# yuriyvnv/speech_transcript_embeddings

Measured on AMD Instinct MI355X. Metric: audio–text pairs/sec (whole node), 10s@16kHz + 64-tok, 1/2/4/8 MI355X, higher is better.
Workload: dtype bf16; 1 GPU; c2: global batch 64 = 1 GPU x 1 micro-batch(es) of 64 pairs, each pair 10s@16kHz audio + 64-tok clean + 64-tok corrupt; w2v-bert-2.0 Conformer 24L + XLM-R-base 12L, 3+3 unfrozen; GPU fbank -> fwd -> InfoNCE -> bwd -> allreduce -> clip+AdamW; global_batch=64, local_batch=64, micro_batch=64, accumulation_steps=1, seq_len_audio_frames=499, seq_len_text=64, parallelism=dp1

## Files before the change

include/ste.h:

```cpp
#ifndef STE_H_
#define STE_H_
#include <stdint.h>

#ifdef __cplusplus
extern "C" {
#endif

#define STE_OK 0
#define STE_ERR_ARG 1001
#define STE_ERR_SHAPE 1002

enum {
  STE_ACT_NONE = 0,
  STE_ACT_SWISH = 1,
  STE_ACT_GELU = 2,
  STE_ACT_TANH = 3,
  STE_ACT_RELU = 4,
  STE_ACT_SWISH_BWD = 11,
  STE_ACT_GELU_BWD = 12,
  STE_ACT_TANH_BWD_OUT = 13,
  STE_ACT_RELU_BWD = 14
};

typedef struct {
// ... 61 lines not shown
  const void* dy; int64_t lddy; int dy_bf16;
  const void* x; int64_t ldx; int x_bf16;
  const float* mean; const float* rstd;
  const float* gamma; const float* beta;
  const float* row_scale;
  int act;
  const float* dres; int64_t lddres;
  float* dx; int64_t lddx;
  void* dxb; int64_t lddxb;
  float* dgamma; float* dbeta;
  float drop_p; uint64_t seed; float out_scale;
  float in_drop_p; uint64_t in_seed;
  const float* out_row_scale;
  float* dsum;
  float* ws; int64_t ws_floats;
} ste_ln_bwd_args;
int ste_layernorm_bwd(const ste_ln_bwd_args* a, void* stream);
int64_t ste_layernorm_bwd_ws_floats(int rows, int cols);

int ste_layernorm_fwd_pair(const ste_ln_fwd_args* a, const ste_ln_fwd_args* b, void* stream);
int ste_layernorm_bwd_pair(const ste_ln_bwd_args* a, const ste_ln_bwd_args* b, void* stream);

typedef struct {
  int B, T, H;
  const void* q; int64_t ldq;
  const void* k; int64_t ldk;
  const void* v; int64_t ldv;
  void* o; int64_t ldo;
  float* lse;
  const int32_t* key_mask;
  const void* rel_E; int rel_left, rel_right;
  float scale;
  float drop_p; uint64_t seed;
  const void* dout; int64_t lddo;
  void* dq; int64_t lddq;
  void* dk; int64_t lddk;
  void* dv; int64_t lddv;
  float* delta;
  float* dE;
  float* gwork;
  void* o_lo; int64_t ldolo;
  int zero_masked_rows;
} ste_attn_args;
int ste_attention_fwd(const ste_attn_args* a, void* stream);
int ste_attention_fwd_f32(const ste_attn_args* a, float* o32, int64_t ldo32, void* stream);
int ste_attention_bwd(const ste_attn_args* a, void* stream);
int ste_attention_bwd_f32(const ste_attn_args* a, void* stream);

int ste_glu_dwconv_fwd(const void* pre, const float* w, void* out, int B, int T, int C, int K, void* stream);
int ste_glu_dwconv_bwd(const void* pre, const float* w, const void* dout, void* dpre, float* dw,
                       int B, int T, int C, int K, float* ws, int64_t ws_floats, void* stream);
int64_t ste_glu_dwconv_bwd_ws_floats(int B, int T, int C, int K);

int ste_fbank(const float* wav, int64_t ld_wav, const int32_t* lengths, int B, int Tmax, float pad_value,
              float* feats, int64_t* mask, int mask_mode, float* work, void* stream);

int ste_resample_plan(int sr_in, int sr_out, int* M, int* L, int* K);
int ste_resample_table(int sr_in, int sr_out, float* table, int64_t table_floats);
int ste_resample_tile(int M, int L, int K);
int ste_resample(const float* wav, int64_t ld_wav, const int32_t* lengths, int B, int M, int L, int K,
                 const float* table, float* out, int64_t ld_out, int n_out_max, int32_t* out_lengths, void* stream);

int ste_attn_pool_fwd(const void* t, const float* w2, const float* b2, const void* h, const int32_t* mask,
                      int B, int L, int Hh, int H, float* weights, float* pooled, void* pooled_bf16,
                      void* stream);
int ste_attn_pool_bwd_work_floats(int B, int L, int Hh);
int ste_attn_pool_bwd(const void* t, const float* w2, const void* h, const float* weights, const float* dpooled,
                      const int32_t* mask, int B, int L, int Hh, int H, float* dh, void* dt, void* dt_lo, float* dw2,
                      float* db2,
                      float* db1, float* work, void* stream);
int ste_attn_pool_fwd_f32(const float* t, const float* w2, const float* b2, const float* h, const int32_t* mask,
                          int B, int L, int Hh, int H, float* weights, float* pooled, void* pooled_bf16, void* stream);
int ste_attn_pool_bwd_f32(const float* t, const float* w2, const float* h, const float* weights, const float* dpooled,
                          const int32_t* mask, int B, int L, int Hh, int H, float* dh, float* dt, float* dw2,
                          float* db2, float* db1, float* work, void* stream);

int ste_mean_pool_fwd(const void* h, const int32_t* mask, int B, int L, int H, int cls, float* weights, float* pooled,
                      void* pooled_bf16, void* stream);
int ste_mean_pool_fwd_f32(const float* h, const int32_t* mask, int B, int L, int H, int cls, float* weights,
                          float* pooled, void* pooled_bf16, void* stream);
int ste_weighted_pool_bwd(const float* weights, const float* dpooled, int B, int L, int H, float* dh, void* stream);

int ste_xattn1_fwd(const float* q, const void* k, const void* v, int64_t ldkv, const int32_t* mask, int B, int S,
                   int P, int nh, float scale, float drop_p, uint64_t seed, float* probs, float* out, void* stream);
int ste_xattn1_bwd(const float* q, const void* k, const void* v, int64_t ldkv, const float* probs, const float* dout,
                   const int32_t* mask, int B, int S, int P, int nh, float scale, float drop_p, uint64_t seed,
                   float* dq, float* dk, float* dv, int64_t lddkv, void* stream);
int ste_xattn_fwd(const float* q, const void* k, const void* v, int64_t ldkv, const int32_t* mask, int B, int S, int P,
                  int nh, int nq, float scale, float drop_p, uint64_t seed0, uint64_t seed1, float* probs, float* out,
                  void* stream);
int ste_xattn_bwd(const float* q, const void* k, const void* v, int64_t ldkv, const float* probs, const float* dout,
                  const int32_t* mask, int B, int S, int P, int nh, int nq, float scale, float drop_p,
                  uint64_t seed0, uint64_t seed1, float* dq, float* dk, float* dv, int64_t lddkv, void* stream);
int ste_xattn_mq_fwd(const float* q, const int32_t* qrow, const void* k, const void* v, int64_t ldkv,
                     const int32_t* mask, int B, int C, int S, int P, int nh, float scale, float* out, void* stream);
int ste_xattn_gather_fwd(const float* q, const int32_t* qrow, const void* k, const void* v, int64_t ldkv,
                         const int32_t* kvblk, const int32_t* mask, int R, int S, int P, int nh, float scale,
                         float* out, void* stream);
int ste_xattn_seg_fwd(const float* q, const int32_t* qrow, const int32_t* pseg, const void* k, const void* v,
                      int64_t ldkv, const int64_t* seg_row, const int32_t* seg_len, const int32_t* tile_first,
                      const int32_t* tile_cnt, int ntile, int R, int G, int P, int nh, float scale, float* out,
                      void* stream);
int ste_xattn_seg_mx8_fwd(const float* q, const int32_t* qrow, const int32_t* pseg, const void* k, const void* v,
                          int64_t ldkv, const void* ks, const void* vs, int64_t lds, const int64_t* seg_row,
                          const int32_t* seg_len, const int32_t* tile_first, const int32_t* tile_cnt, int ntile,
                          int R, int G, int P, int nh, float scale, float* out, void* stream);
// ... 140 lines not shown
```

speech_transcript_embeddings_amd/_lib.py:

```python
from __future__ import annotations

import ctypes as C
import os
from pathlib import Path

import torch

_PKG = Path(__file__).resolve().parent
LIB_PATH = Path(os.environ.get("STE_LIB", _PKG / "libste.so"))
AB_BUILD = LIB_PATH.name == "libste_ab.so"


def ab_env(name: str, default: str) -> str:
    return os.environ.get(name, default) if AB_BUILD else default

c_void_p, c_int, c_int64, c_float, c_uint64, c_char_p = C.c_void_p, C.c_int, C.c_int64, C.c_float, C.c_uint64, C.c_char_p
c_i32p = C.POINTER(C.c_int32)

ACT_NONE, ACT_SWISH, ACT_GELU, ACT_TANH, ACT_RELU = 0, 1, 2, 3, 4
ACT_SWISH_BWD, ACT_GELU_BWD, ACT_TANH_BWD_OUT, ACT_RELU_BWD = 11, 12, 13, 14


class GemmArgs(C.Structure):
    _fields_ = [
# ... 58 lines not shown
    _fields_ = [
        ("B", c_int), ("T", c_int), ("H", c_int),
        ("q", c_void_p), ("ldq", c_int64),
        ("k", c_void_p), ("ldk", c_int64),
        ("v", c_void_p), ("ldv", c_int64),
        ("o", c_void_p), ("ldo", c_int64),
        ("lse", c_void_p),
        ("key_mask", c_void_p),
        ("rel_E", c_void_p), ("rel_left", c_int), ("rel_right", c_int),
        ("scale", c_float),
        ("drop_p", c_float), ("seed", c_uint64),
        ("dout", c_void_p), ("lddo", c_int64),
        ("dq", c_void_p), ("lddq", c_int64),
        ("dk", c_void_p), ("lddk", c_int64),
        ("dv", c_void_p), ("lddv", c_int64),
        ("delta", c_void_p),
        ("dE", c_void_p),
        ("gwork", c_void_p),
        ("o_lo", c_void_p), ("ldolo", c_int64),
        ("zero_masked_rows", c_int),
    ]


_SIGS = {
    "ste_gemm": (c_int, [C.POINTER(GemmArgs), c_void_p]),
    "ste_gemm_f32": (c_int, [C.POINTER(GemmArgs), c_void_p]),
    "ste_gemm_f32_plan": (c_int, [C.POINTER(GemmArgs)]),
    "ste_gemm_f32_plan_slab": (c_int, [C.POINTER(GemmArgs)]),
    "ste_gemm_f32_ws_floats": (c_int64, [C.POINTER(GemmArgs)]),
    "ste_gemm_f32_plan_max_tiles": (c_int, [c_int]),
    "ste_gemm_f32_plan_small_tiles": (c_int, [c_int]),
    "ste_gemm_f32_plan_tile": (c_int, [C.POINTER(GemmArgs)]),
    "ste_gemm_kernel": (c_int, [C.POINTER(GemmArgs)]),
    "ste_gemm_colsum_ws_floats": (c_int64, [C.POINTER(GemmArgs)]),
    "ste_gemm_tile_map": (c_int, [c_int, c_int, c_int, C.POINTER(c_int), C.POINTER(c_int)]),
    "ste_gemm_kernel_name": (c_int, [C.POINTER(GemmArgs), c_char_p, c_int]),
    "ste_rows_extract": (c_int, [c_void_p, c_int, c_int, c_void_p, c_int, c_void_p, c_void_p, c_void_p, c_int,
                                 c_void_p, c_void_p]),
    "ste_rows_accumulate": (c_int, [c_void_p, c_int, c_void_p, c_void_p, c_int, c_float, c_void_p]),
    "ste_layernorm_fwd": (c_int, [C.POINTER(LnFwdArgs), c_void_p]),
    "ste_layernorm_bwd": (c_int, [C.POINTER(LnBwdArgs), c_void_p]),
    "ste_layernorm_fwd_pair": (c_int, [C.POINTER(LnFwdArgs), C.POINTER(LnFwdArgs), c_void_p]),
    "ste_layernorm_bwd_pair": (c_int, [C.POINTER(LnBwdArgs), C.POINTER(LnBwdArgs), c_void_p]),
    "ste_layernorm_bwd_ws_floats": (c_int64, [c_int, c_int]),
    "ste_attention_fwd": (c_int, [C.POINTER(AttnArgs), c_void_p]),
    "ste_attention_bwd": (c_int, [C.POINTER(AttnArgs), c_void_p]),
    "ste_attention_fwd_f32": (c_int, [C.POINTER(AttnArgs), c_void_p, c_int64, c_void_p]),
    "ste_attention_bwd_f32": (c_int, [C.POINTER(AttnArgs), c_void_p]),
    "ste_split_bf16": (c_int, [c_void_p, c_int64, c_int64, c_int, c_void_p, c_int, c_int, c_void_p]),
    "ste_glu_dwconv_fwd": (c_int, [c_void_p, c_void_p, c_void_p, c_int, c_int, c_int, c_int, c_void_p]),
    "ste_glu_dwconv_bwd": (c_int, [c_void_p, c_void_p, c_void_p, c_void_p, c_void_p, c_int, c_int, c_int, c_int,
                                   c_void_p, c_int64, c_void_p]),
    "ste_glu_dwconv_bwd_ws_floats": (c_int64, [c_int, c_int, c_int, c_int]),
    "ste_fbank": (c_int, [c_void_p, c_int64, c_void_p, c_int, c_int, c_float, c_void_p, c_void_p, c_int, c_void_p,
                          c_void_p]),
    "ste_resample_plan": (c_int, [c_int, c_int, C.POINTER(c_int), C.POINTER(c_int), C.POINTER(c_int)]),
    "ste_resample_table": (c_int, [c_int, c_int, c_void_p, c_int64]),
    "ste_resample_tile": (c_int, [c_int, c_int, c_int]),
    "ste_resample": (c_int, [c_void_p, c_int64, c_void_p, c_int, c_int, c_int, c_int, c_void_p, c_void_p, c_int64,
                             c_int, c_void_p, c_void_p]),
    "ste_gemm_mx8": (c_int, [c_void_p, c_void_p, c_void_p, c_void_p, c_void_p, c_void_p]),
    "ste_gemm_mx8_kernel": (c_int, [C.POINTER(GemmArgs), c_int]),
    "ste_gemm_plan_min_tiles": (c_int, [c_int, c_int, C.POINTER(c_int), C.POINTER(c_int)]),
    "ste_mx8_quant": (c_int, [c_void_p, c_int64, c_int, c_int, c_void_p, c_void_p, c_void_p]),
    "ste_mx8_dequant": (c_int, [c_void_p, c_int64, c_int, c_int, c_void_p, c_void_p, c_void_p]),
    "ste_attn_pool_fwd": (c_int, [c_void_p, c_void_p, c_void_p, c_void_p, c_void_p, c_int, c_int, c_int, c_int,
                                  c_void_p, c_void_p, c_void_p, c_void_p]),
    "ste_attn_pool_bwd": (c_int, [c_void_p, c_void_p, c_void_p, c_void_p, c_void_p, c_void_p, c_int, c_int, c_int,
                                  c_int, c_void_p, c_void_p, c_void_p, c_void_p, c_void_p, c_void_p, c_void_p,
                                  c_void_p]),
    "ste_attn_pool_bwd_work_floats": (c_int, [c_int, c_int, c_int]),
    "ste_attn_pool_fwd_f32": (c_int, [c_void_p, c_void_p, c_void_p, c_void_p, c_void_p, c_int, c_int, c_int, c_int,
                                      c_void_p, c_void_p, c_void_p, c_void_p]),
    "ste_attn_pool_bwd_f32": (c_int, [c_void_p, c_void_p, c_void_p, c_void_p, c_void_p, c_void_p, c_int, c_int,
                                      c_int, c_int, c_void_p, c_void_p, c_void_p, c_void_p, c_void_p, c_void_p,
                                      c_void_p]),
    "ste_mean_pool_fwd": (c_int, [c_void_p, c_void_p, c_int, c_int, c_int, c_int, c_void_p, c_void_p, c_void_p,
                                  c_void_p]),
    "ste_mean_pool_fwd_f32": (c_int, [c_void_p, c_void_p, c_int, c_int, c_int, c_int, c_void_p, c_void_p, c_void_p,
                                      c_void_p]),
    "ste_weighted_pool_bwd": (c_int, [c_void_p, c_void_p, c_int, c_int, c_int, c_void_p, c_void_p]),
    "ste_xattn1_fwd": (c_int, [c_void_p, c_void_p, c_void_p, c_int64, c_void_p, c_int, c_int, c_int, c_int, c_float,
                               c_float, c_uint64, c_void_p, c_void_p, c_void_p]),
    "ste_xattn1_bwd": (c_int, [c_void_p, c_void_p, c_void_p, c_int64, c_void_p, c_void_p, c_void_p, c_int, c_int,
                               c_int, c_int, c_float, c_float, c_uint64, c_void_p, c_void_p, c_void_p, c_int64,
                               c_void_p]),
    "ste_xattn_fwd": (c_int, [c_void_p, c_void_p, c_void_p, c_int64, c_void_p, c_int, c_int, c_int, c_int, c_int,
                              c_float, c_float, c_uint64, c_uint64, c_void_p, c_void_p, c_void_p]),
    "ste_xattn_bwd": (c_int, [c_void_p, c_void_p, c_void_p, c_int64, c_void_p, c_void_p, c_void_p, c_int, c_int,
                              c_int, c_int, c_int, c_float, c_float, c_uint64, c_uint64, c_void_p, c_void_p,
                              c_void_p, c_int64, c_void_p]),
    "ste_xattn_bwd_bf16": (c_int, [c_void_p, c_void_p, c_void_p, c_int64, c_void_p, c_void_p, c_void_p, c_int,
                                   c_int, c_int, c_int, c_int, c_float, c_float, c_uint64, c_uint64, c_void_p,
                                   c_void_p, c_void_p, c_int64, c_void_p, c_void_p]),
    "ste_xattn_mq_fwd": (c_int, [c_void_p, c_void_p, c_void_p, c_void_p, c_int64, c_void_p, c_int, c_int, c_int,
                                 c_int, c_int, c_float, c_void_p, c_void_p]),
    "ste_xattn_gather_fwd": (c_int, [c_void_p, c_void_p, c_void_p, c_void_p, c_int64, c_void_p, c_void_p, c_int,
                                     c_int, c_int, c_int, c_float, c_void_p, c_void_p]),
    "ste_xattn_seg_fwd": (c_int, [c_void_p, c_void_p, c_void_p, c_void_p, c_void_p, c_int64, c_void_p, c_void_p,
                                  c_void_p, c_void_p, c_int, c_int, c_int, c_int, c_int, c_float, c_void_p,
                                  c_void_p]),
    "ste_xattn_seg_mx8_fwd": (c_int, [c_void_p, c_void_p, c_void_p, c_void_p, c_void_p, c_int64, c_void_p, c_void_p,
                                      c_int64, c_void_p, c_void_p, c_void_p, c_void_p, c_int, c_int, c_int, c_int,
                                      c_int, c_float, c_void_p, c_void_p]),
    "ste_align_attn_fwd": (c_int, [c_void_p, c_int64, c_void_p, c_int64, c_void_p, c_int, c_int, c_int, c_int, c_int,
                                   c_float, c_uint64, c_void_p, c_void_p, c_int64, c_void_p]),
# ... 138 lines not shown
```

speech_transcript_embeddings_amd/csrc/layernorm.hip:

```cpp
#include "common.h"
#include "../../include/ste.h"

namespace {

constexpr int NT = 256;

template <int MAXC>
STE_DEV void load_row(const void* base, bool is_bf16, int64_t ld, int row, int cols, int lane, float (&v)[MAXC * 4]) {
#pragma unroll
  for (int c = 0; c < MAXC; ++c) {
    int col = (lane + c * 64) * 4;
    f32x4 x = {0.f, 0.f, 0.f, 0.f};
    if (col < cols) {
      if (is_bf16) x = load_bf16x4((const bf16*)base + (int64_t)row * ld + col);
      else x = *reinterpret_cast<const f32x4*>((const float*)base + (int64_t)row * ld + col);
    }
#pragma unroll
    for (int e = 0; e < 4; ++e) v[c * 4 + e] = x[e];
  }
}

template <int MAXC>
struct LnParams {
  f32x4 g[MAXC], b[MAXC];
  STE_DEV void load(const float* gamma, const float* beta, int cols, int lane) {
#pragma unroll
    for (int c = 0; c < MAXC; ++c) {
      const int col = (lane + c * 64) * 4;
      g[c] = col < cols ? *reinterpret_cast<const f32x4*>(gamma + col) : f32x4{0.f, 0.f, 0.f, 0.f};
      b[c] = (beta && col < cols) ? *reinterpret_cast<const f32x4*>(beta + col) : f32x4{0.f, 0.f, 0.f, 0.f};
    }
  }
};

template <int MAXC>
STE_DEV void ln_fwd_row(const ste_ln_fwd_args& a, const LnParams<MAXC>& pr, int row, int lane, float (&v)[MAXC * 4]) {
  const float inv_n = 1.0f / (float)a.cols;
  const uint32_t thresh = (uint32_t)(a.drop_p * 4294967296.0);
  const float inv_keep = a.drop_p > 0.f ? 1.0f / (1.0f - a.drop_p) : 1.0f;
  float s = 0.f;
#pragma unroll
  for (int i = 0; i < MAXC * 4; ++i) s += v[i];
  const float mean = wave_sum(s) * inv_n;
  float q = 0.f;
#pragma unroll
  for (int c = 0; c < MAXC; ++c) {
    int col = (lane + c * 64) * 4;
    if (col < a.cols) {
#pragma unroll
      for (int e = 0; e < 4; ++e) { float d = v[c * 4 + e] - mean; q += d * d; }
    }
  }
  const float rstd = rsqrtf(wave_sum(q) * inv_n + a.eps);
  if (lane == 0) { a.mean[row] = mean; a.rstd[row] = rstd; }
  const float rs = a.row_scale ? a.row_scale[row] : 1.0f;
#pragma unroll
  for (int c = 0; c < MAXC; ++c) {
    int col = (lane + c * 64) * 4;
    if (col >= a.cols) continue;
    const f32x4 g = pr.g[c], b = pr.b[c];
    f32x4 y;
#pragma unroll
    for (int e = 0; e < 4; ++e) {
      float t = ((v[c * 4 + e] - mean) * rstd * g[e] + b[e]) * rs;
      if (a.act == STE_ACT_SWISH) t = swish_f(t);
      if (a.drop_p > 0.f) t *= drop_scale(a.seed, (uint64_t)row * a.cols + col + e, thresh, inv_keep);
      y[e] = t;
      v[c * 4 + e] = t;
    }
    if (a.y) *reinterpret_cast<f32x4*>(a.y + (int64_t)row * a.ldy + col) = y;
    if (a.ylo) store_bf16x4_split((bf16*)a.yb + (int64_t)row * a.ldyb + col, (bf16*)a.ylo + (int64_t)row * a.ldylo + col, y);
    else if (a.yb) store_bf16x4((bf16*)a.yb + (int64_t)row * a.ldyb + col, y);
    if (a.q8) {
      float am = fmaxf(fmaxf(fabsf(y[0]), fabsf(y[1])), fmaxf(fabsf(y[2]), fabsf(y[3])));
      am = fmaxf(am, dpp_f<0xB1>(am));
      am = fmaxf(am, dpp_f<0x4E>(am));
      am = fmaxf(am, dpp_f<0x141>(am));
      const int ex = mx8_exp(am);
      const float inv = ldexpf(1.0f, -ex);
      uint32_t w = 0;
      w = __builtin_amdgcn_cvt_pk_fp8_f32(fminf(fmaxf(y[0] * inv, -448.f), 448.f),
                                          fminf(fmaxf(y[1] * inv, -448.f), 448.f), w, false);
      w = __builtin_amdgcn_cvt_pk_fp8_f32(fminf(fmaxf(y[2] * inv, -448.f), 448.f),
                                          fminf(fmaxf(y[3] * inv, -448.f), 448.f), w, true);
      *reinterpret_cast<uint32_t*>((uint8_t*)a.q8 + (int64_t)row * a.ldq8 + col) = w;
      if ((lane & 7) == 0) ((uint8_t*)a.q8s)[(int64_t)row * (a.cols >> 5) + (col >> 5)] = (uint8_t)(ex + 127);
    }
  }
}

template <int MAXC>
__global__ __launch_bounds__(NT) void ln_fwd_kernel(ste_ln_fwd_args a) {
  const int lane = threadIdx.x & 63;
  const int wave = blockIdx.x * (NT / 64) + (threadIdx.x >> 6);
  const int nwaves = gridDim.x * (NT / 64);
  LnParams<MAXC> pa;
  pa.load(a.gamma, a.beta, a.cols, lane);
  for (int row = wave; row < a.rows; row += nwaves) {
    float v[MAXC * 4];
    load_row<MAXC>(a.x, a.x_bf16, a.ldx, row, a.cols, lane, v);
    ln_fwd_row<MAXC>(a, pa, row, lane, v);
  }
}

template <int MAXC, bool LEAN = false>
__global__ __launch_bounds__(NT) void ln_fwd_pair_kernel(ste_ln_fwd_args a, ste_ln_fwd_args b) {
  const int lane = threadIdx.x & 63;
  const int wave = blockIdx.x * (NT / 64) + (threadIdx.x >> 6);
  const int nwaves = gridDim.x * (NT / 64);
  if constexpr (LEAN) {
    for (int row = wave; row < a.rows; row += nwaves) {
      float v[MAXC * 4];
      load_row<MAXC>(a.x, a.x_bf16, a.ldx, row, a.cols, lane, v);
      const float *ga = a.gamma, *ba = a.beta, *gb = b.gamma, *bb = b.beta;
      asm volatile("" : "+s"(ga), "+s"(ba), "+s"(gb), "+s"(bb));
      {
        LnParams<MAXC> pa;
        pa.load(ga, ba, a.cols, lane);
        ln_fwd_row<MAXC>(a, pa, row, lane, v);
      }
      LnParams<MAXC> pb;
      pb.load(gb, bb, b.cols, lane);
      ln_fwd_row<MAXC>(b, pb, row, lane, v);
    }
  } else {
    LnParams<MAXC> pa;
    pa.load(a.gamma, a.beta, a.cols, lane);
    LnParams<MAXC> pb;
    pb.load(b.gamma, b.beta, b.cols, lane);
    float v[MAXC * 4], nx[MAXC * 4];
    if (wave < a.rows) load_row<MAXC>(a.x, a.x_bf16, a.ldx, wave, a.cols, lane, v);
    for (int row = wave; row < a.rows; row += nwaves) {
      if (row + nwaves < a.rows) load_row<MAXC>(a.x, a.x_bf16, a.ldx, row + nwaves, a.cols, lane, nx);
      ln_fwd_row<MAXC>(a, pa, row, lane, v);
      ln_fwd_row<MAXC>(b, pb, row, lane, v);
#pragma unroll
      for (int i = 0; i < MAXC * 4; ++i) v[i] = nx[i];
    }
  }
}
// ... 304 lines not shown
```

speech_transcript_embeddings_amd/engine.py:

```python
from __future__ import annotations

import math

import torch

from . import _lib, ops
from ._lib import (ACT_GELU, ACT_GELU_BWD, ACT_NONE, ACT_RELU, ACT_RELU_BWD, ACT_SWISH, ACT_SWISH_BWD,
                   ACT_TANH)

BF16, F32 = torch.bfloat16, torch.float32
_GOLD = 0x9E3779B97F4A7C15
_M64 = (1 << 64) - 1


def _site_seed(base: int, site: int) -> int:
    x = (base + (site + 1) * _GOLD) & _M64
    x ^= x >> 31
    return (x * 0xBF58476D1CE4E5B9) & _M64


XLMR_NAMES = dict(layer="text_encoder.encoder.layer.{i}.", q="attention.self.query", o="attention.output.dense",
                  ln1="attention.output.LayerNorm", fi="intermediate.dense", fo="output.dense", ln2="output.LayerNorm")
W2V2_NAMES = dict(layer="audio_encoder.encoder.layers.{i}.", q="attention.q_proj", o="attention.out_proj",
                  ln1="layer_norm", fi="feed_forward.intermediate_dense", fo="feed_forward.output_dense",
                  ln2="final_layer_norm")


class Ctx(dict):
    """Saved activations of one forward (freed when backward finishes)."""


class Engine:
    def __init__(self, model):
        self.m = model
        self.s = model.store
        self.acfg = model.audio_cfg
        self.tcfg = model.text_cfg
        self._ws = {}
        self._side = None
        self.overlap = _lib.ab_env("STE_TEXT_STREAM", "1") != "0"
        self.layerdrop_gen = None
        self.ln_pair = _lib.ab_env("STE_LN_PAIR", "1") != "0"
        self.text_after_first_layer = _lib.ab_env("STE_TEXT_AFTER_LAYER", "1") != "0"
        self.precise_text = _lib.ab_env("STE_TEXT_PRECISE", "1") != "0"
        self.precise_text_bwd = _lib.ab_env("STE_TEXT_PRECISE_BWD", "0") == "1"

    @property
    def fp8(self):
        return bool(getattr(self.m, "fp8_gemm", False))

    @property
    def fp8_bwd(self):
        return self.fp8 and bool(getattr(self.m, "fp8_bwd", False))

    WS_BYTES = 80 << 20

    @property
    def ws(self):
        return ops.stream_ws(self.s.device, self.WS_BYTES // 4, cache=self._ws)

    def _await_params(self, *names):
        evs = getattr(self, "param_events", None)
        if evs:
            cur = torch.cuda.current_stream(self.s.device)
            for n in names:
                ev = evs.get(n)
                if ev is not None:
                    cur.wait_event(ev)

    def _side_stream(self):
        if not (self.overlap and self.s.device.type == "cuda"):
            return None
        if self._side is None:
            self._side = torch.cuda.Stream(device=self.s.device)
        return self._side

    def _e(self, *shape, dtype=F32):
        return torch.empty(shape, device=self.s.device, dtype=dtype)

    def _z(self, *shape, dtype=F32):
        return torch.zeros(shape, device=self.s.device, dtype=dtype)

    def _dw(self, dy_b, x_b, wname, fused=1):
        g = self.s.fused(wname, fused, "g")
        if g is None:
            return
        g2 = g.view(g.shape[0], -1)
        ops.linear_dw(dy_b, x_b, out=g2, beta=1.0, ws=self.ws)

    def _dx(self, dy, wname, fused=1, **kw):
        kw.setdefault("ws", self.ws)
        return ops.linear(dy, self.s.wt(wname, fused), **kw)

    def _dx_mx8(self, dy, wname, fused=1, **kw):
        kw.pop("ws", None)
# ... 90 lines not shown
                xq = xb if isinstance(xb, tuple) else ops.mx8_quant(xb)
                return ops.linear_mx8(xq, s.wq(wname, count), bias, **kw)
            return ops.linear(xb, s.fused(wname, count, "w"), bias, **kw)

        def ffn_in(a, wname, bname, z):
            if not fp8:
                h = lin(a, wname, s.p(bname), act=ACT_SWISH, pre_out=z, out_bf16=True)
                return h, h
            q = (self._e(M, F_, dtype=torch.uint8), self._e(M, F_ // 32, dtype=torch.uint8))
            h = self._e(M, F_, dtype=BF16) if (tr and save) else False
            lin(a, wname, s.p(bname), act=ACT_SWISH, pre_out=z, out=h, out_bf16=True, q_out=q)
            return (h if h is not False else None), q

        def ln_in(xin, name, st, **kw):
            if not fp8:
                y = self._e(M, D, dtype=BF16)
                sv[st] = self._ln(xin, name, eps, yb=y, **kw)
                return y, y
            y = self._e(M, D, dtype=BF16) if (tr and save) else None
            q = (self._e(M, D, dtype=torch.uint8), self._e(M, D // 32, dtype=torch.uint8))
            sv[st] = self._ln(xin, name, eps, yb=y, q8=q, **kw)
            return y, q

        def ln_in_out(name, tr_, **kw):
            if not fp8:
                y = self._e(M, D, dtype=BF16)
                return dict(yb=y, **kw), y, y
            y = self._e(M, D, dtype=BF16) if (tr_ and save) else None
            q = (self._e(M, D, dtype=torch.uint8), self._e(M, D // 32, dtype=torch.uint8))
            return dict(yb=y, q8=q, **kw), y, q

        if pre1 is not None:
            a1, a1in, sv["st1"] = pre1
        else:
            a1, a1in = ln_in(x, pre + "ffn1_layer_norm", "st1")
        z1 = self._e(M, F_, dtype=BF16) if save else None
        h1, h1in = ffn_in(a1in, pre + "ffn1.intermediate_dense.weight", pre + "ffn1.intermediate_dense.bias", z1)
        x1 = lin(h1in, pre + "ffn1.output_dense.weight", s.p(pre + "ffn1.output_dense.bias"), alpha=0.5,
                 residual=x)
        a2, a2in = ln_in(x1, pre + "self_attn_layer_norm", "st2")
        qkv = lin(a2in, pre + "self_attn.linear_q.weight", s.fused(pre + "self_attn.linear_q.bias", 3, "p"), count=3,
                  out_bf16=True)
        o = self._e(M, D, dtype=BF16)
        o_lo = self._e(M, D, dtype=BF16) if save else None
        lse = self._e(b * H * T)
        ops.attention_fwd(qkv[:, :D], qkv[:, D:2 * D], qkv[:, 2 * D:], B=b, T=T, H=H, o=o, lse=lse, key_mask=mask32,
                          rel_E=s.w(pre + "self_attn.distance_embedding.weight"),
                          rel_left=c.left_max_position_embeddings, rel_right=c.right_max_position_embeddings,
                          scale=1.0 / math.sqrt(D // H), o_lo=o_lo)
        x2 = lin(o, pre + "self_attn.linear_out.weight", s.p(pre + "self_attn.linear_out.bias"), residual=x1)
        a3, a3in = ln_in(x2, pre + "conv_module.layer_norm", "st3", row_scale=maskf)
        pw1 = lin(a3in, pre + "conv_module.pointwise_conv1.weight", None, out_bf16=True)
        cv = self._e(M, D, dtype=BF16)
        ops.glu_dwconv_fwd(pw1, s.p(pre + "conv_module.depthwise_conv.weight").view(D, -1), cv, b, T)
        sw, swin = ln_in(cv, pre + "conv_module.depthwise_layer_norm", "st4", act=ACT_SWISH)
        p_conv = c.conformer_conv_dropout if train else 0.0
        x3 = lin(swin, pre + "conv_module.pointwise_conv2.weight", None, residual=x2, drop_p=p_conv,
                 seed=_site_seed(seed, 1))
        a5, a5in = ln_in(x3, pre + "ffn2_layer_norm", "st5")
        z2 = self._e(M, F_, dtype=BF16) if save else None
        h2, h2in = ffn_in(a5in, pre + "ffn2.intermediate_dense.weight", pre + "ffn2.intermediate_dense.bias", z2)
        x4 = lin(h2in, pre + "ffn2.output_dense.weight", s.p(pre + "ffn2.output_dense.bias"), alpha=0.5,
                 residual=x3)
        x5 = self._e(M, D)
        x5s = self._e(M, 2 * D, dtype=BF16) if want_bf16 else None
        x5b = x5s[:, :D] if want_bf16 else None
        x5lo = x5s[:, D:] if want_bf16 else None
        pre_next = None
        if nxt is None:
            sv["st6"] = self._ln(x4, pre + "final_layer_norm", eps, y=x5, yb=x5b, ylo=x5lo)
        else:
            prej = f"audio_encoder.encoder.layers.{nxt}.ffn1_layer_norm"
            trj = s.trainable_layer(f"audio_encoder.encoder.layers.{nxt}.ffn1_layer_norm.weight")
            second, a1j, a1inj = ln_in_out(prej, trj, gamma=s.p(prej + ".weight"), beta=s.p(prej + ".bias"), eps=eps)
            sv["st6"], st1j = ops.layernorm_fwd_pair(
                dict(x=x4, gamma=s.p(pre + "final_layer_norm.weight"), beta=s.p(pre + "final_layer_norm.bias"), eps=eps,
                     y=x5, yb=x5b, ylo=x5lo), second)
            pre_next = (a1j, a1inj, st1j)
        sv.update(x=x, z1=z1, x1=x1, qkv=qkv, o=o, o_lo=o_lo, lse=lse, x2=x2, pw1=pw1, cv=cv, x3=x3, z2=z2, x4=x4, p_conv=p_conv)
        if tr:
            sv.update(a1=a1, h1=h1, a2=a2, a3=a3, sw=sw, a5=a5, h2=h2)
        return x5, x5s, sv, pre_next

    def _ln_bwd_kw(self, x, stats, name, **kw):
        return dict(x=x, mean=stats[0], rstd=stats[1], gamma=self.s.p(name + ".weight"), beta=self.s.p(name + ".bias"),
                    dgamma=self.s.g(name + ".weight"), dbeta=self.s.g(name + ".bias"), **kw)

    def _conformer_bwd(self, i, sv, dx5, b, T, maskf, mask32, pending=None):
        c = self.acfg
        s = self.s
        pre = f"audio_encoder.encoder.layers.{i}."
        M, D, F_ = sv["x4"].shape[0], c.hidden_size, c.intermediate_size
        H = c.num_attention_heads
        tr = sv["tr"]
        _dx = self._dx_mx8 if self.fp8_bwd else self._dx
        dx4 = self._e(M, D)
        dx4b = self._e(M, D, dtype=BF16)
        if pending is None:
            self._ln_bwd(dx5, sv["x4"], sv["st6"], pre + "final_layer_norm", dx=dx4, dxb=dx4b, out_scale=0.5,
                         dsum=s.g(pre + "ffn2.output_dense.bias"))
        else:
            ops.layernorm_bwd_pair(self._ln_bwd_kw(sv["x4"], sv["st6"], pre + "final_layer_norm", dx=dx4, dxb=dx4b,
                                                   out_scale=0.5, dsum=s.g(pre + "ffn2.output_dense.bias")), pending)
        dz2 = _dx(dx4b, pre + "ffn2.output_dense.weight", act=ACT_SWISH_BWD, z=sv["z2"],
                            out_bf16=True, colsum=s.g(pre + "ffn2.intermediate_dense.bias"))
        if tr:
            self._dw(dx4b, sv["h2"], pre + "ffn2.output_dense.weight")
        da5 = _dx(dz2, pre + "ffn2.intermediate_dense.weight", out_bf16=True)
# ... 1057 lines not shown
```

speech_transcript_embeddings_amd/ops.py:

```python
from __future__ import annotations

import ctypes as C
import os

import torch

from . import _lib
from ._lib import GemmArgs, LnFwdArgs, LnBwdArgs, AttnArgs, ptr, call, fn

BF16 = torch.bfloat16
F32 = torch.float32


def _s():
    return _lib.stream_ptr()


def _ld(t: torch.Tensor) -> int:
    assert t.dim() >= 2 and t.stride(-1) == 1, "row-major operand required"
    return t.stride(-2)


ATOMIC_SUMS = _lib.ab_env("STE_ATOMIC_SUMS", "0") == "1"
_WS = {}
# ... 370 lines not shown
    a.dv, a.lddv = ptr(dv), _ld(dv)
    call("ste_attention_bwd_f32", C.byref(a), _s())


def split_bf16(x, nblk, lo_mask, out=None):
    rows, K = x.shape
    if out is None:
        out = torch.empty((rows, nblk * K), device=x.device, dtype=BF16)
    assert out.shape == (rows, nblk * K) and out.is_contiguous() and out.dtype == BF16
    call("ste_split_bf16", ptr(x), _ld(x), rows, K, ptr(out), int(nblk), int(lo_mask), _s())
    return out


def linear_x2(x, w2, bias=None, **kw):
    return gemm(split_bf16(x, 2, 2), w2, a_kc=True, b_kc=True, bias=bias, **kw)


def attention_bwd(q, k, v, o, lse, dout, dq, dk, dv, *, B, T, H, delta, key_mask=None, rel_E=None, rel_left=64,
                  rel_right=8, scale=0.125, drop_p=0.0, seed=0, dE=None, gwork=None, o_lo=None):
    a = AttnArgs()
    a.B, a.T, a.H = B, T, H
    a.q, a.ldq = ptr(q), _ld(q)
    a.k, a.ldk = ptr(k), _ld(k)
    a.v, a.ldv = ptr(v), _ld(v)
    a.o, a.ldo = ptr(o), _ld(o)
    a.lse = ptr(lse)
    a.key_mask = ptr(key_mask)
    a.rel_E, a.rel_left, a.rel_right = ptr(rel_E), rel_left, rel_right
    a.scale, a.drop_p, a.seed = float(scale), float(drop_p), int(seed) & (2**64 - 1)
    a.dout, a.lddo = ptr(dout), _ld(dout)
    a.dq, a.lddq = ptr(dq), _ld(dq)
    a.dk, a.lddk = ptr(dk), _ld(dk)
    a.dv, a.lddv = ptr(dv), _ld(dv)
    a.delta, a.dE, a.gwork = ptr(delta), ptr(dE), ptr(gwork)
    if o_lo is not None:
        a.o_lo, a.ldolo = ptr(o_lo), _ld(o_lo)
    call("ste_attention_bwd", C.byref(a), _s())


def glu_dwconv_fwd(pre, w, out, B, T):
    C_ = w.shape[0]
    call("ste_glu_dwconv_fwd", ptr(pre), ptr(w), ptr(out), B, T, C_, w.shape[-1], _s())
    return out


def glu_dwconv_bwd(pre, w, dout, dpre, dw, B, T):
    C_ = w.shape[0]
    ws = _red_ws(pre.device, int(fn("ste_glu_dwconv_bwd_ws_floats")(B, T, C_, w.shape[-1]))) if dw is not None else None
    call("ste_glu_dwconv_bwd", ptr(pre), ptr(w), ptr(dout), ptr(dpre), ptr(dw), B, T, C_, w.shape[-1], *_ws_args(ws),
         _s())
    return dpre


def fbank(wav, lengths, Tmax, *, pad_value=1.0, mask_mode=0, feats=None, mask=None, work=None):
    B = wav.shape[0]
    dev = wav.device
    if feats is None:
        feats = torch.empty((B, Tmax, 160), device=dev, dtype=F32)
    if mask is None:
        mask = torch.empty((B, Tmax), device=dev, dtype=torch.int64)
    if work is None:
        work = torch.empty(B * 2 * Tmax * 80 + B * 160, device=dev, dtype=F32)
    nbytes = 4 * B * wav.shape[1] + _nb(feats) + _nb(mask)
    _traced("fbank", nbytes, lambda: call("ste_fbank", ptr(wav), wav.stride(0), ptr(lengths), B, Tmax,
                                          float(pad_value), ptr(feats), ptr(mask), int(mask_mode), ptr(work), _s()))
    return feats, mask


def resample_plan(sr_in, sr_out=16000):
    M, L, K = C.c_int(), C.c_int(), C.c_int()
    call("ste_resample_plan", int(sr_in), int(sr_out), C.byref(M), C.byref(L), C.byref(K))
    return M.value, L.value, K.value


def resampled_length(n, sr_in, sr_out=16000):
    if sr_in == sr_out:
        return int(n)
    M, L, _ = resample_plan(sr_in, sr_out)
    return (int(n) * L + M - 1) // M


def resample_tile(sr_in, sr_out=16000):
    return fn("ste_resample_tile")(*resample_plan(sr_in, sr_out))


_RESAMPLE_TABLES = {}


def _resample_table(sr_in, sr_out, dev):
    key = (int(sr_in), int(sr_out), dev)
    t = _RESAMPLE_TABLES.get(key)
    if t is None:
        _, L, K = resample_plan(sr_in, sr_out)
        host = torch.empty(L * K, dtype=F32)
        call("ste_resample_table", int(sr_in), int(sr_out), host.data_ptr(), host.numel())
        t = _RESAMPLE_TABLES[key] = host.to(dev)
    return t


def resample(wav, lengths, sr_in, sr_out=16000, *, out=None):
    if int(sr_in) == int(sr_out):
        return wav, lengths
    M, L, K = resample_plan(sr_in, sr_out)
    B, N = wav.shape
    dev = wav.device
    if not wav.is_cuda or lengths.device != dev or lengths.shape != (B,):
# ... 425 lines not shown
```

Baseline: 491.7 pairs/s.

## Fuse GLU depthwise conv with swish layernorm in conformer forward

Adds a fused HIP kernel that computes GLU plus the 31-tap depthwise convolution over a sliding register window, stages output rows in double-buffered LDS, and applies the depthwise layernorm with swish per row in the same kernel. The aim is to avoid re-reading the conv output from global memory for a separate layernorm launch and to drop one kernel launch per conformer layer. The layernorm row routine moves into a shared header so both kernels use it. The fused path still writes cv for backward, is gated on shape and block count, and is off under fp8.

Measured after the change: 490.9 pairs/s. No clear change (-0.2%).

```diff
diff --git a/include/ste.h b/include/ste.h
--- a/include/ste.h
+++ b/include/ste.h
@@ -137,6 +137,10 @@
                        int B, int T, int C, int K, float* ws, int64_t ws_floats, void* stream);
 int64_t ste_glu_dwconv_bwd_ws_floats(int B, int T, int C, int K);
 
+int ste_conv_ln_plan(int B, int T, int C, int* R, int* blocks, int* threads, int* lds_bytes);
+int ste_glu_dwconv_ln_fwd(const void* pre, const float* w, void* cv, const ste_ln_fwd_args* ln, int B, int T, int K,
+                          int R, void* stream);
+
 int ste_fbank(const float* wav, int64_t ld_wav, const int32_t* lengths, int B, int Tmax, float pad_value,
               float* feats, int64_t* mask, int mask_mode, float* work, void* stream);
 
diff --git a/profiles/conv_ln_probe.py b/profiles/conv_ln_probe.py
--- /dev/null
+++ b/profiles/conv_ln_probe.py
@@ -0,0 +1,111 @@
+import argparse
+import json
+import os
+import statistics
+import sys
+
+import torch
+
+ROOT = os.path.dirname(os.path.dirname(os.path.abspath(__file__)))
+sys.path.insert(0, ROOT)
+BF16 = torch.bfloat16
+SWISH = 1
+
+
+def main():
+    ap = argparse.ArgumentParser()
+    ap.add_argument("--shapes", default="64x499x1024")
+    ap.add_argument("--runs", default="64,128,256")
+    ap.add_argument("--iters", type=int, default=24)
+    ap.add_argument("--repeats", type=int, default=5)
+    ap.add_argument("--sets", type=int, default=3)
+    ap.add_argument("--out", default=os.path.join(ROOT, "profiles", "conv_ln_probe.json"))
+    args = ap.parse_args()
+    from speech_transcript_embeddings_amd import ops
+    dev = "cuda:0"
+    runs = [0] + [int(r) for r in args.runs.split(",")]
+
+    def timed(launch):
+        for k in range(args.sets):
+            launch(k)
+        torch.cuda.synchronize()
+        graph = torch.cuda.CUDAGraph()
+        with torch.cuda.graph(graph):
+            for i in range(args.iters):
+                launch(i % args.sets)
+        graph.replay()
+        torch.cuda.synchronize()
+        us = []
+        for _ in range(args.repeats):
+            e0, e1 = torch.cuda.Event(enable_timing=True), torch.cuda.Event(enable_timing=True)
+            e0.record()
+            graph.replay()
+            e1.record()
+            torch.cuda.synchronize()
+            us.append(e0.elapsed_time(e1) * 1e3 / args.iters)
+        return {"us": round(statistics.median(us), 2), "min": round(min(us), 2), "max": round(max(us), 2)}
+
+    def with_rate(t, nbytes):
+        t["GBps"] = round(nbytes / t["us"] * 1e-3, 1)
+        return t
+
+    result = {"timing": "graph replay", "iters": args.iters, "repeats": args.repeats, "sets": args.sets, "shapes": {}}
+    for shape in args.shapes.split(","):
+        B, T, D = (int(v) for v in shape.split("x"))
+        M = B * T
+        g = torch.Generator(device=dev).manual_seed(0)
+        sets = []
+        for _ in range(args.sets):
+            s = dict(pw1=torch.randn(M, 2 * D, device=dev, generator=g).to(BF16),
+                     cv=torch.empty(M, D, device=dev, dtype=BF16), sw=torch.empty(M, D, device=dev, dtype=BF16),
+                     mean=torch.empty(M, device=dev), rstd=torch.empty(M, device=dev))
+            sets.append(s)
+        w = 0.25 * torch.randn(D, 31, device=dev, generator=g)
+        gamma = 1.0 + 0.3 * torch.randn(D, device=dev, generator=g)
+        beta = 0.3 * torch.randn(D, device=dev, generator=g)
+
+        def conv_fwd(k):
+            s = sets[k]
+            ops.glu_dwconv_fwd(s["pw1"], w, s["cv"], B, T)
+
+        def ln_fwd(k):
+            s = sets[k]
+            ops.layernorm_fwd(s["cv"], gamma, beta, 1e-5, yb=s["sw"], mean=s["mean"], rstd=s["rstd"], act=SWISH)
+
+        def fused_fwd(R):
+            def f(k):
+                s = sets[k]
+                ops.glu_dwconv_ln_fwd(s["pw1"], w, s["cv"], gamma, beta, 1e-5, s["sw"], B, T, mean=s["mean"],
+                                      rstd=s["rstd"], R=R)
+            return f
+
+        for f in (conv_fwd, ln_fwd):
+            f(0)
+        ref = {k: sets[0][k].clone() for k in ("cv", "sw", "mean", "rstd")}
+        equal = {}
+        for R in runs:
+            for k in ("cv", "sw", "mean", "rstd"):
+                sets[0][k].fill_(float("nan"))
+            fused_fwd(R)(0)
+            equal[str(R)] = all(torch.equal(sets[0][k].view(torch.int16 if sets[0][k].dtype == BF16 else torch.int32),
+                                            ref[k].view(torch.int16 if ref[k].dtype == BF16 else torch.int32)) for k in ref)
+        e = 2
+        b_conv_f, b_ln_f = M * D * e * 3, M * D * e * 2 + 8 * M
+        b_fused_f = M * D * e * 4 + 8 * M
+        d = {"B": B, "T": T, "D": D, "plan": ops.conv_ln_plan(B, T, D), "bitwise_equal": equal,
+             "glu_dwconv_fwd": with_rate(timed(conv_fwd), b_conv_f), "layernorm_fwd": with_rate(timed(ln_fwd), b_ln_f),
+             "glu_dwconv_ln_fwd": {}}
+        d["pair_fwd_us"] = round(d["glu_dwconv_fwd"]["us"] + d["layernorm_fwd"]["us"], 2)
+        for R in runs:
+            rr = R or d["plan"]["R"]
+            blocks = B * ((T + rr - 1) // rr)
+            d["glu_dwconv_ln_fwd"][str(R)] = dict(with_rate(timed(fused_fwd(R)), b_fused_f), R=rr, blocks=blocks)
+        result["shapes"][shape] = d
+        print(json.dumps(d), flush=True)
+        del sets
+    with open(args.out, "w") as f:
+        json.dump(result, f, indent=1)
+
+
+if __name__ == "__main__":
+    main()
diff --git a/speech_transcript_embeddings_amd/_lib.py b/speech_transcript_embeddings_amd/_lib.py
--- a/speech_transcript_embeddings_amd/_lib.py
+++ b/speech_transcript_embeddings_amd/_lib.py
@@ -134,6 +134,10 @@
     "ste_glu_dwconv_bwd": (c_int, [c_void_p, c_void_p, c_void_p, c_void_p, c_void_p, c_int, c_int, c_int, c_int,
                                    c_void_p, c_int64, c_void_p]),
     "ste_glu_dwconv_bwd_ws_floats": (c_int64, [c_int, c_int, c_int, c_int]),
+    "ste_conv_ln_plan": (c_int, [c_int, c_int, c_int, C.POINTER(c_int), C.POINTER(c_int), C.POINTER(c_int),
+                                 C.POINTER(c_int)]),
+    "ste_glu_dwconv_ln_fwd": (c_int, [c_void_p, c_void_p, c_void_p, C.POINTER(LnFwdArgs), c_int, c_int, c_int, c_int,
+                                      c_void_p]),
     "ste_fbank": (c_int, [c_void_p, c_int64, c_void_p, c_int, c_int, c_float, c_void_p, c_void_p, c_int, c_void_p,
                           c_void_p]),
     "ste_resample_plan": (c_int, [c_int, c_int, C.POINTER(c_int), C.POINTER(c_int), C.POINTER(c_int)]),
diff --git a/speech_transcript_embeddings_amd/csrc/conv_ln.hip b/speech_transcript_embeddings_amd/csrc/conv_ln.hip
--- /dev/null
+++ b/speech_transcript_embeddings_amd/csrc/conv_ln.hip
@@ -0,0 +1,141 @@
+#include "common.h"
+#include "ln_rows.h"
+#include "../../include/ste.h"
+
+namespace {
+
+using namespace ste_ln;
+
+typedef __bf16 bf16x2 __attribute__((ext_vector_type(2)));
+
+constexpr int K = 31;
+constexpr int CH = 8;
+constexpr int NUM_CU = 256;
+
+STE_DEV float glu1(bf16 a, bf16 g) { return (float)a * sigmoidf_((float)g); }
+
+STE_DEV void load_pair(const bf16* __restrict__ clip, uint32_t c2, int t, int T, int D, bf16x2& av, bf16x2& gv) {
+  const bool ok = t >= 0 && t < T;
+  const bf16* row = clip + (int64_t)(ok ? t : 0) * (2 * D);
+  const bf16x2 x = *reinterpret_cast<const bf16x2*>(row + c2), y = *reinterpret_cast<const bf16x2*>(row + D + c2);
+  av = ok ? x : bf16x2{};
+  gv = ok ? y : bf16x2{};
+}
+
+template <int MAXC>
+__global__ __launch_bounds__(MAXC * 128) void glu_dwconv_ln_fwd_kernel(const bf16* __restrict__ pre,
+                                                                     const float* __restrict__ w,
+                                                                     bf16* __restrict__ cv, ste_ln_fwd_args a, int T,
+                                                                     int R) {
+  __shared__ bf16 rows[2][CH][MAXC * 256];
+  const int D = a.cols;
+  const int tid = threadIdx.x, lane = tid & 63, wave = tid >> 6, nw = blockDim.x >> 6;
+  const int b = blockIdx.y, t0 = blockIdx.x * R, tend = min(t0 + R, T);
+  const uint32_t c2 = 2 * tid;
+  float wk0[K], wk1[K];
+#pragma unroll
+  for (int k = 0; k < K; ++k) {
+    wk0[k] = w[c2 * K + k];
+    wk1[k] = w[(c2 + 1) * K + k];
+  }
+  const bf16* clip = pre + (int64_t)b * T * (2 * D);
+  float win0[K - 1 + CH], win1[K - 1 + CH];
+  {
+    bf16x2 ha[K - 1], hg[K - 1];
+#pragma unroll
+    for (int j = 0; j < K - 1; ++j) load_pair(clip, c2, t0 - (K - 1) + j, T, D, ha[j], hg[j]);
+#pragma unroll
+    for (int j = 0; j < K - 1; ++j) {
+      win0[j] = glu1(ha[j][0], hg[j][0]);
+      win1[j] = glu1(ha[j][1], hg[j][1]);
+    }
+  }
+  bf16x2 na[CH], ng[CH];
+#pragma unroll
+  for (int i = 0; i < CH; ++i) load_pair(clip, c2, t0 + i, tend, D, na[i], ng[i]);
+  for (int n = 0, tc = t0; tc < tend; ++n, tc += CH) {
+#pragma unroll
+    for (int i = 0; i < CH; ++i) {
+      win0[K - 1 + i] = glu1(na[i][0], ng[i][0]);
+      win1[K - 1 + i] = glu1(na[i][1], ng[i][1]);
+    }
+#pragma unroll
+    for (int i = 0; i < CH; ++i) load_pair(clip, c2, tc + CH + i, tend, D, na[i], ng[i]);
+    float acc0[CH], acc1[CH];
+#pragma unroll
+    for (int i = 0; i < CH; ++i) acc0[i] = acc1[i] = 0.f;
+#pragma unroll
+    for (int k = 0; k < K; ++k)
+#pragma unroll
+      for (int i = 0; i < CH; ++i) {
+        acc0[i] += wk0[k] * win0[i + k];
+        acc1[i] += wk1[k] * win1[i + k];
+      }
+    bf16 (*buf)[MAXC * 256] = rows[n & 1];
+#pragma unroll
+    for (int i = 0; i < CH; ++i) {
+      bf16x2 o;
+      o[0] = (bf16)acc0[i];
+      o[1] = (bf16)acc1[i];
+      *reinterpret_cast<bf16x2*>(&buf[i][c2]) = o;
+    }
+#pragma unroll
+    for (int j = 0; j < K - 1; ++j) {
+      win0[j] = win0[j + CH];
+      win1[j] = win1[j + CH];
+    }
+    __syncthreads();
+    for (int r = wave; r < CH; r += nw) {
+      const int t = tc + r;
+      if (t >= tend) break;
+      const int row = b * T + t;
+      float v[MAXC * 4];
+#pragma unroll
+      for (int c = 0; c < MAXC; ++c) {
+        const int col = (lane + c * 64) * 4;
+        bf16x4 x = bf16x4{};
+        if (col < D) {
+          x = *reinterpret_cast<const bf16x4*>(&buf[r][col]);
+          *reinterpret_cast<bf16x4*>(cv + (int64_t)row * D + col) = x;
+        }
+#pragma unroll
+        for (int e = 0; e < 4; ++e) v[c * 4 + e] = (float)x[e];
+      }
+      const LnParamsRef pr{{a.gamma, lane}, {a.beta, lane}};
+      ln_fwd_row<MAXC>(a, pr, row, lane, v);
+    }
+  }
+}
+
+int plan_rows(int B, int T) { return (int64_t)B * ((T + 127) / 128) >= NUM_CU ? 128 : 64; }
+bool shape_ok(int B, int T, int D, int Kw) {
+  return B > 0 && T > 0 && D > 0 && D <= 1024 && (D % 256) == 0 && Kw == K && (int64_t)B * T <= 0x7fffffff;
+}
+
+}
+
+extern "C" int ste_conv_ln_plan(int B, int T, int D, int* R, int* blocks, int* threads, int* lds_bytes) {
+  if (!shape_ok(B, T, D, K)) return STE_ERR_SHAPE;
+  const int r = plan_rows(B, T);
+  if (R) *R = r;
+  if (blocks) *blocks = B * ((T + r - 1) / r);
+  if (threads) *threads = D / 2;
+  if (lds_bytes) *lds_bytes = 2 * CH * (D <= 256 ? 256 : 1024) * (int)sizeof(bf16);
+  return 0;
+}
+
+extern "C" int ste_glu_dwconv_ln_fwd(const void* pre, const float* w, void* cv, const ste_ln_fwd_args* ln, int B,
+                                     int T, int Kw, int R, void* stream) {
+  if (!pre || !w || !cv || !ln || !ln->yb || !ln->mean || !ln->rstd || !ln->gamma || !ln->beta) return STE_ERR_ARG;
+  if (ln->y || ln->ylo || ln->q8 || ln->ldyb < ln->cols) return STE_ERR_ARG;
+  if (!shape_ok(B, T, ln->cols, Kw) || (int64_t)ln->rows != (int64_t)B * T) return STE_ERR_SHAPE;
+  if (R == 0) R = plan_rows(B, T);
+  if (R < CH || (R % CH) != 0) return STE_ERR_ARG;
+  const int D = ln->cols;
+  const dim3 grid((T + R - 1) / R, B), block(D / 2);
+  hipStream_t s = (hipStream_t)stream;
+  if (D <= 256) hipLaunchKernelGGL(glu_dwconv_ln_fwd_kernel<1>, grid, block, 0, s, (const bf16*)pre, w, (bf16*)cv, *ln, T, R);
+  else hipLaunchKernelGGL(glu_dwconv_ln_fwd_kernel<4>, grid, block, 0, s, (const bf16*)pre, w, (bf16*)cv, *ln, T, R);
+  STE_CHECK_LAUNCH();
+  return 0;
+}
diff --git a/speech_transcript_embeddings_amd/csrc/layernorm.hip b/speech_transcript_embeddings_amd/csrc/layernorm.hip
--- a/speech_transcript_embeddings_amd/csrc/layernorm.hip
+++ b/speech_transcript_embeddings_amd/csrc/layernorm.hip
@@ -1,7 +1,10 @@
 #include "common.h"
+#include "ln_rows.h"
 #include "../../include/ste.h"
 
 namespace {
+
+using namespace ste_ln;
 
 constexpr int NT = 256;
 
@@ -17,75 +20,6 @@
     }
 #pragma unroll
     for (int e = 0; e < 4; ++e) v[c * 4 + e] = x[e];
-  }
-}
-
-template <int MAXC>
-struct LnParams {
-  f32x4 g[MAXC], b[MAXC];
-  STE_DEV void load(const float* gamma, const float* beta, int cols, int lane) {
-#pragma unroll
-    for (int c = 0; c < MAXC; ++c) {
-      const int col = (lane + c * 64) * 4;
-      g[c] = col < cols ? *reinterpret_cast<const f32x4*>(gamma + col) : f32x4{0.f, 0.f, 0.f, 0.f};
-      b[c] = (beta && col < cols) ? *reinterpret_cast<const f32x4*>(beta + col) : f32x4{0.f, 0.f, 0.f, 0.f};
-    }
-  }
-};
-
-template <int MAXC>
-STE_DEV void ln_fwd_row(const ste_ln_fwd_args& a, const LnParams<MAXC>& pr, int row, int lane, float (&v)[MAXC * 4]) {
-  const float inv_n = 1.0f / (float)a.cols;
-  const uint32_t thresh = (uint32_t)(a.drop_p * 4294967296.0);
-  const float inv_keep = a.drop_p > 0.f ? 1.0f / (1.0f - a.drop_p) : 1.0f;
-  float s = 0.f;
-#pragma unroll
-  for (int i = 0; i < MAXC * 4; ++i) s += v[i];
-  const float mean = wave_sum(s) * inv_n;
-  float q = 0.f;
-#pragma unroll
-  for (int c = 0; c < MAXC; ++c) {
-    int col = (lane + c * 64) * 4;
-    if (col < a.cols) {
-#pragma unroll
-      for (int e = 0; e < 4; ++e) { float d = v[c * 4 + e] - mean; q += d * d; }
-    }
-  }
-  const float rstd = rsqrtf(wave_sum(q) * inv_n + a.eps);
-  if (lane == 0) { a.mean[row] = mean; a.rstd[row] = rstd; }
-  const float rs = a.row_scale ? a.row_scale[row] : 1.0f;
-#pragma unroll
-  for (int c = 0; c < MAXC; ++c) {
-    int col = (lane + c * 64) * 4;
-    if (col >= a.cols) continue;
-    const f32x4 g = pr.g[c], b = pr.b[c];
-    f32x4 y;
-#pragma unroll
-    for (int e = 0; e < 4; ++e) {
-      float t = ((v[c * 4 + e] - mean) * rstd * g[e] + b[e]) * rs;
-      if (a.act == STE_ACT_SWISH) t = swish_f(t);
-      if (a.drop_p > 0.f) t *= drop_scale(a.seed, (uint64_t)row * a.cols + col + e, thresh, inv_keep);
-      y[e] = t;
-      v[c * 4 + e] = t;
-    }
-    if (a.y) *reinterpret_cast<f32x4*>(a.y + (int64_t)row * a.ldy + col) = y;
-    if (a.ylo) store_bf16x4_split((bf16*)a.yb + (int64_t)row * a.ldyb + col, (bf16*)a.ylo + (int64_t)row * a.ldylo + col, y);
-    else if (a.yb) store_bf16x4((bf16*)a.yb + (int64_t)row * a.ldyb + col, y);
-    if (a.q8) {
-      float am = fmaxf(fmaxf(fabsf(y[0]), fabsf(y[1])), fmaxf(fabsf(y[2]), fabsf(y[3])));
-      am = fmaxf(am, dpp_f<0xB1>(am));
-      am = fmaxf(am, dpp_f<0x4E>(am));
-      am = fmaxf(am, dpp_f<0x141>(am));
-      const int ex = mx8_exp(am);
-      const float inv = ldexpf(1.0f, -ex);
-      uint32_t w = 0;
-      w = __builtin_amdgcn_cvt_pk_fp8_f32(fminf(fmaxf(y[0] * inv, -448.f), 448.f),
-                                          fminf(fmaxf(y[1] * inv, -448.f), 448.f), w, false);
-      w = __builtin_amdgcn_cvt_pk_fp8_f32(fminf(fmaxf(y[2] * inv, -448.f), 448.f),
-                                          fminf(fmaxf(y[3] * inv, -448.f), 448.f), w, true);
-      *reinterpret_cast<uint32_t*>((uint8_t*)a.q8 + (int64_t)row * a.ldq8 + col) = w;
-      if ((lane & 7) == 0) ((uint8_t*)a.q8s)[(int64_t)row * (a.cols >> 5) + (col >> 5)] = (uint8_t)(ex + 127);
-    }
   }
 }
 
diff --git a/speech_transcript_embeddings_amd/csrc/ln_rows.h b/speech_transcript_embeddings_amd/csrc/ln_rows.h
--- /dev/null
+++ b/speech_transcript_embeddings_amd/csrc/ln_rows.h
@@ -0,0 +1,84 @@
+#pragma once
+#include "common.h"
+#include "../../include/ste.h"
+
+namespace ste_ln {
+
+template <int MAXC>
+struct LnParams {
+  f32x4 g[MAXC], b[MAXC];
+  STE_DEV void load(const float* gamma, const float* beta, int cols, int lane) {
+#pragma unroll
+    for (int c = 0; c < MAXC; ++c) {
+      const int col = (lane + c * 64) * 4;
+      g[c] = col < cols ? *reinterpret_cast<const f32x4*>(gamma + col) : f32x4{0.f, 0.f, 0.f, 0.f};
+      b[c] = (beta && col < cols) ? *reinterpret_cast<const f32x4*>(beta + col) : f32x4{0.f, 0.f, 0.f, 0.f};
+    }
+  }
+};
+
+struct LnParamsRef {
+  struct Vec {
+    const float* p;
+    int lane;
+    STE_DEV f32x4 operator[](int c) const { return *reinterpret_cast<const f32x4*>(p + (lane + c * 64) * 4); }
+  } g, b;
+};
+
+template <int MAXC, class P>
+STE_DEV void ln_fwd_row(const ste_ln_fwd_args& a, const P& pr, int row, int lane, float (&v)[MAXC * 4]) {
+  const float inv_n = 1.0f / (float)a.cols;
+  const uint32_t thresh = (uint32_t)(a.drop_p * 4294967296.0);
+  const float inv_keep = a.drop_p > 0.f ? 1.0f / (1.0f - a.drop_p) : 1.0f;
+  float s = 0.f;
+#pragma unroll
+  for (int i = 0; i < MAXC * 4; ++i) s += v[i];
+  const float mean = wave_sum(s) * inv_n;
+  float q = 0.f;
+#pragma unroll
+  for (int c = 0; c < MAXC; ++c) {
+    int col = (lane + c * 64) * 4;
+    if (col < a.cols) {
+#pragma unroll
+      for (int e = 0; e < 4; ++e) { float d = v[c * 4 + e] - mean; q += d * d; }
+    }
+  }
+  const float rstd = rsqrtf(wave_sum(q) * inv_n + a.eps);
+  if (lane == 0) { a.mean[row] = mean; a.rstd[row] = rstd; }
+  const float rs = a.row_scale ? a.row_scale[row] : 1.0f;
+#pragma unroll
+  for (int c = 0; c < MAXC; ++c) {
+    int col = (lane + c * 64) * 4;
+    if (col >= a.cols) continue;
+    const f32x4 g = pr.g[c], b = pr.b[c];
+    f32x4 y;
+#pragma unroll
+    for (int e = 0; e < 4; ++e) {
+      float t = ((v[c * 4 + e] - mean) * rstd * g[e] + b[e]) * rs;
+      if (a.act == STE_ACT_SWISH) t = swish_f(t);
+      if (a.drop_p > 0.f) t *= drop_scale(a.seed, (uint64_t)row * a.cols + col + e, thresh, inv_keep);
+      y[e] = t;
+      v[c * 4 + e] = t;
+    }
+    if (a.y) *reinterpret_cast<f32x4*>(a.y + (int64_t)row * a.ldy + col) = y;
+    if (a.ylo) store_bf16x4_split((bf16*)a.yb + (int64_t)row * a.ldyb + col, (bf16*)a.ylo + (int64_t)row * a.ldylo + col, y);
+    else if (a.yb) store_bf16x4((bf16*)a.yb + (int64_t)row * a.ldyb + col, y);
+    if (a.q8) {
+      float am = fmaxf(fmaxf(fabsf(y[0]), fabsf(y[1])), fmaxf(fabsf(y[2]), fabsf(y[3])));
+      am = fmaxf(am, dpp_f<0xB1>(am));
+      am = fmaxf(am, dpp_f<0x4E>(am));
+      am = fmaxf(am, dpp_f<0x141>(am));
+      const int ex = mx8_exp(am);
+      const float inv = ldexpf(1.0f, -ex);
+      uint32_t w = 0;
+      w = __builtin_amdgcn_cvt_pk_fp8_f32(fminf(fmaxf(y[0] * inv, -448.f), 448.f),
+                                          fminf(fmaxf(y[1] * inv, -448.f), 448.f), w, false);
+      w = __builtin_amdgcn_cvt_pk_fp8_f32(fminf(fmaxf(y[2] * inv, -448.f), 448.f),
+                                          fminf(fmaxf(y[3] * inv, -448.f), 448.f), w, true);
+      *reinterpret_cast<uint32_t*>((uint8_t*)a.q8 + (int64_t)row * a.ldq8 + col) = w;
+      if ((lane & 7) == 0) ((uint8_t*)a.q8s)[(int64_t)row * (a.cols >> 5) + (col >> 5)] = (uint8_t)(ex + 127);
+    }
+  }
+}
+
+}
diff --git a/speech_transcript_embeddings_amd/engine.py b/speech_transcript_embeddings_amd/engine.py
--- a/speech_transcript_embeddings_amd/engine.py
+++ b/speech_transcript_embeddings_amd/engine.py
@@ -41,6 +41,8 @@
         self.overlap = _lib.ab_env("STE_TEXT_STREAM", "1") != "0"
         self.layerdrop_gen = None
         self.ln_pair = _lib.ab_env("STE_LN_PAIR", "1") != "0"
+        self.conv_ln_fused = _lib.ab_env("STE_CONV_LN", "1") != "0"
+        self.conv_ln_min_blocks = 256
         self.text_after_first_layer = _lib.ab_env("STE_TEXT_AFTER_LAYER", "1") != "0"
         self.precise_text = _lib.ab_env("STE_TEXT_PRECISE", "1") != "0"
         self.precise_text_bwd = _lib.ab_env("STE_TEXT_PRECISE_BWD", "0") == "1"
@@ -237,8 +239,15 @@
         a3, a3in = ln_in(x2, pre + "conv_module.layer_norm", "st3", row_scale=maskf)
         pw1 = lin(a3in, pre + "conv_module.pointwise_conv1.weight", None, out_bf16=True)
         cv = self._e(M, D, dtype=BF16)
-        ops.glu_dwconv_fwd(pw1, s.p(pre + "conv_module.depthwise_conv.weight").view(D, -1), cv, b, T)
-        sw, swin = ln_in(cv, pre + "conv_module.depthwise_layer_norm", "st4", act=ACT_SWISH)
+        wdw = s.p(pre + "conv_module.depthwise_conv.weight").view(D, -1)
+        if (self.conv_ln_fused and not fp8 and D <= 1024 and D % 256 == 0
+                and b * ((T + 127) // 128) >= self.conv_ln_min_blocks):
+            dln = pre + "conv_module.depthwise_layer_norm"
+            sw = swin = self._e(M, D, dtype=BF16)
+            sv["st4"] = ops.glu_dwconv_ln_fwd(pw1, wdw, cv, s.p(dln + ".weight"), s.p(dln + ".bias"), eps, sw, b, T)
+        else:
+            ops.glu_dwconv_fwd(pw1, wdw, cv, b, T)
+            sw, swin = ln_in(cv, pre + "conv_module.depthwise_layer_norm", "st4", act=ACT_SWISH)
         p_conv = c.conformer_conv_dropout if train else 0.0
         x3 = lin(swin, pre + "conv_module.pointwise_conv2.weight", None, residual=x2, drop_p=p_conv,
                  seed=_site_seed(seed, 1))
diff --git a/speech_transcript_embeddings_amd/ops.py b/speech_transcript_embeddings_amd/ops.py
--- a/speech_transcript_embeddings_amd/ops.py
+++ b/speech_transcript_embeddings_amd/ops.py
@@ -446,6 +446,21 @@
     return dpre
 
 
+def conv_ln_plan(B, T, D):
+    out = [C.c_int() for _ in range(4)]
+    call("ste_conv_ln_plan", B, T, D, *(C.byref(o) for o in out))
+    return dict(zip(("R", "blocks", "threads", "lds_bytes"), (o.value for o in out)))
+
+
+def glu_dwconv_ln_fwd(pre, w, cv, gamma, beta, eps, yb, B, T, *, mean=None, rstd=None, act=_lib.ACT_SWISH, R=0):
+    a, mean, rstd, _ = _ln_fwd_struct(None, gamma, beta, eps, yb=yb, mean=mean, rstd=rstd, act=act, rows=B * T,
+                                      cols=w.shape[0])
+    nbytes = _nb(pre) + _nb(cv) + _nb(yb) + 8 * B * T + _nb(w) + 8 * w.shape[0]
+    _traced("glu_dwconv_ln_fwd", nbytes, lambda: call("ste_glu_dwconv_ln_fwd", ptr(pre), ptr(w), ptr(cv), C.byref(a),
+                                                      B, T, w.shape[-1], R, _s()))
+    return mean, rstd
+
+
 def fbank(wav, lengths, Tmax, *, pad_value=1.0, mask_mode=0, feats=None, mask=None, work=None):
     B = wav.shape[0]
     dev = wav.device
```
